# NVlabs/DREAM

Hardware: AMD Instinct MI355X
Metric: frames/s DREAM-vgg-q 400x400 b=128 inference (higher is better)
Workload: dtype f32

## Files before the change

dream_amd/csrc/conv_wino4.hip:

```cpp
#include <type_traits>
#include <stdlib.h>
#include <dream_cdna4.h>
#include "common.h"
#include "pack_device.h"
#include "../../include/dream_hip.h"

#ifndef DREAM_W4_DIAG
#define DREAM_W4_DIAG 0
#endif

namespace {

struct Wino4Params {
    const float *x;
    const float *u;
    const float *scale;
    const float *shift;
    const float *residual;
    float *y;
    float *y_full;
    int B, H, W, Cin, Cout, CoutPad;
    int TY, TX;
    int ntiles;
    int nblk, blk_per_xcd;
    unsigned long long magic_tpi, magic_tx;
    int flags;
    int out_scale, out_oy, out_ox;
    int in_scale, in_oy, in_ox;
    int stagger_n, stagger_unit;
    int ymap;
};

constexpr int W4T = 16;
constexpr int W4P = 36;
#ifndef DREAM_W4_RING
#define DREAM_W4_RING 8
#endif
#ifndef DREAM_W4_NARROW_RING
#define DREAM_W4_NARROW_RING 18
#endif
#ifndef DREAM_W4_PAT_RING
#define DREAM_W4_PAT_RING 10
#endif
#ifndef DREAM_W4_PAT_S1OFF
#define DREAM_W4_PAT_S1OFF 8
#endif
#ifndef DREAM_W4_S1
#define DREAM_W4_S1 10
#define DREAM_W4_S2 13
#define DREAM_W4_LX 3
#endif


template <bool NARROW>
struct W4Cfg {
    static constexpr int NW = NARROW ? 4 : 8;
    static constexpr int K = NARROW ? 8 : 16;
    static constexpr int Q = K / 4;
    static constexpr int KS = K / 4;
    static constexpr int PAD = 16 * NW;
    static constexpr int VPS = NARROW ? W4T * K : W4T * K + 16;
    static constexpr int VB = W4P * VPS;
    static constexpr int SROW = NARROW ? 14 : 25;
    static constexpr int QS = NARROW ? 7 : 6;
    static constexpr int SB = W4T * 6 * SROW * 4;
    static constexpr int RING = NARROW ? DREAM_W4_NARROW_RING : DREAM_W4_RING;
    static constexpr int AHEAD = RING - 2;
    static_assert(72 % RING == 0, "the weight ring must divide two chunks' positions");
    static constexpr bool PAIRS = NARROW && DREAM_W4_NARROW_PAIRS;
    static_assert(!PAIRS || RING % 2 == 0, "a ring of whole pairs");
    using vec = std::conditional_t<NARROW, f32x2, f32x4>;
};
template <bool NARROW>
DREAM_DEVICE int v4_slot(int q, int t) { return NARROW ? q ^ ((t >> 3) & 1) : q ^ ((t >> 2) & 2); }

DREAM_DEVICE f32x4 fma4(float c, f32x4 a, f32x4 b) {
    f32x4 r;
#pragma unroll
    for (int k = 0; k < 4; ++k) r[k] = __builtin_fmaf(c, a[k], b[k]);
    return r;
}

DREAM_DEVICE f32x4 sub4(f32x4 y, f32x4 x) { return pk_sub4(y, x); }
DREAM_DEVICE f32x4 bt_row(int j, const f32x4 *d) {
    switch (j) {
        case 0: return fma4(-2.0f, d[2], fma4(1.5f, sub4(d[3], d[1]), d[0] + d[4]));
        case 1: return fma4(2.5f, d[3], fma4(0.5f, d[2], sub4(d[4], d[1])));
        case 2: return fma4(0.5f, d[3], fma4(-2.5f, d[2], d[4] + d[1]));
        case 3: return fma4(2.0f, sub4(d[3], d[1]), sub4(d[4], d[2]));
        case 4: return fma4(-0.5f, sub4(d[3], d[1]), sub4(d[4], d[2]));
        default: return fma4(-2.0f, d[3], fma4(1.5f, sub4(d[4], d[2]), d[1] + d[5]));
    }
}

DREAM_DEVICE constexpr bool pat4_row_active(int pat, int i) { return pat == 0 || (((pat - 1) >> 1) == 0 ? i <= 4 : i >= 1); }
DREAM_DEVICE constexpr bool pat4_col_active(int pat, int j) { return pat == 0 || (((pat - 1) & 1) == 0 ? j <= 4 : j >= 1); }
DREAM_DEVICE constexpr bool pat4_active(int pat, int pp) { return pat4_row_active(pat, pp / 6) && pat4_col_active(pat, pp % 6); }
DREAM_DEVICE constexpr int pat4_count(int pat) { return pat == 0 ? 36 : 25; }
struct Pat4Table { int pos[36]; };
constexpr Pat4Table pat4_table(int pat) {
    Pat4Table t = {};
    int n = 0;
    for (int pp = 0; pp < 36; ++pp)
        if (pat4_active(pat, pp)) t.pos[n++] = pp;
    return t;
}
template <int PAT>
struct Pat4 { static constexpr Pat4Table table = pat4_table(PAT); };
#define pat4_pos(PAT, k) (Pat4<PAT>::table.pos[k])

template <int MODE, bool NARROW, int PAT = 0>
__global__ void __launch_bounds__(64 * W4Cfg<NARROW>::NW, 2) conv_wino4_kernel(const Wino4Params p) {
    using C = W4Cfg<NARROW>;
    using vec = typename C::vec;
    constexpr int W4K = C::K, W4NW = C::NW, V4PS = C::VPS, V4B = C::VB, S4ROW = C::SROW;
    constexpr int NPOS = pat4_count(PAT);
    constexpr int W4_RING = PAT ? DREAM_W4_PAT_RING : C::RING, W4_AHEAD = W4_RING - 2;
    static_assert((2 * NPOS) % W4_RING == 0, "the weight ring must divide two chunks' positions");
    DREAM_DYNAMIC_LDS(float, sV);
    const int tid = threadIdx.x;
    const int lane = tid & 63;
    const int wave = wave_index();
    const int item_id = wave * 48 + (lane < 48 ? lane : lane - 16);

    const int xcd = (int)(blockIdx.x & 7), J = (int)(gridDim.x >> 3);
    const int part = p.ymap ? xcd / p.ymap : xcd;
    const int blk_hi = (part + 1) * p.blk_per_xcd;
    const int blk_end = blk_hi < p.nblk ? blk_hi : p.nblk;
    int tb = part * p.blk_per_xcd + (int)(blockIdx.x >> 3);
    if (tb >= blk_end) return;
    const int n0 = (p.ymap ? xcd % p.ymap : (int)blockIdx.y) * (16 * W4NW);
    if (p.stagger_n > 1) {
        const unsigned w = blockIdx.x + blockIdx.y * gridDim.x;
        const int naps = (int)((w * 2654435761u >> 16) % (unsigned)p.stagger_n) * p.stagger_unit;
        for (int i = 0; i < naps; ++i) __builtin_amdgcn_s_sleep(127);
    }
    const int tiles_per_img = p.TY * p.TX;
    const int Si = PAT ? p.in_scale : 1;
    const size_t img_floats = (size_t)(Si * p.H) * (Si * p.W) * p.Cin;

    const int q1 = item_id % C::Q, r1 = (item_id / C::Q) % 6, t1 = (item_id / C::Q) / 6;
    const int s1_off = ((t1 * 6 + r1) * S4ROW + C::QS * q1) * 4;
    const int q2 = item_id % C::Q;
    const int j2 = NARROW ? (item_id >> 3) % 6 : (item_id >> 2) % 6;
    const int t2 = NARROW ? 4 * (item_id / 48) + ((item_id >> 1) & 3) : (item_id >> 2) / 6;
    const int s2_off = ((t2 * 6) * S4ROW + C::QS * q2 + j2) * 4;
    const int v2_off = j2 * V4PS + t2 * W4K + 4 * v4_slot<NARROW>(q2, t2);

    unsigned goff0;
    int item1 = t1 | (r1 << 8) | (q1 << 16);
    auto plan_item = [&](int tile0, int b0) {
        asm volatile("" : "+v"(item1));
        const int t = item1 & 255, r = (item1 >> 8) & 255, q = (item1 >> 16) & 255;
        const int tau = tile0 + t;
        const bool tv = tau < p.ntiles;
        const int b = div_magic40(tau, p.magic_tpi), rem = tau - b * tiles_per_img;
        const int ty = div_magic40(rem, p.magic_tx), tx = rem - ty * p.TX;
        const int gy = 4 * ty - 1 + r, x0 = 4 * tx - 1;
        const bool rok = tv & ((unsigned)gy < (unsigned)p.H);
        goff0 = PAT ? (unsigned)(((((b - b0) * Si * p.H + Si * gy + p.in_oy) * (Si * p.W) + Si * x0 + p.in_ox) * p.Cin + 4 * q) * 4)
                    : (unsigned)(((((b - b0) * p.H + gy) * p.W + x0) * p.Cin + 4 * q) * 4);
        item1 &= 0xffffff;
#pragma unroll
        for (int c = 0; c < 6; ++c) item1 |= (rok & ((unsigned)(x0 + c) < (unsigned)p.W)) ? (1 << (24 + c)) : 0;
    };
    const unsigned px_in = (unsigned)(Si * p.Cin * 4);
    auto item_offset = [&](int c) {
        if (DREAM_W4_DIAG & 16) {
            unsigned o = BUFFER_OOB;
            asm volatile("" : "+v"(o));
            return o;
        }
        return (item1 >> (24 + c)) & 1 ? goff0 + (unsigned)c * px_in : BUFFER_OOB;
    };
    auto block_tile0 = [&](int blk) { return blk < blk_end ? blk * W4T : p.ntiles; };
    auto block_xbuf = [&](int b0) {
        return make_buffer(p.x + (size_t)b0 * img_floats, ((size_t)(p.B - b0) * img_floats) * sizeof(float));
    };

    const int lt = lane & 15, lg = lane >> 4;
    const int a_off = NARROW ? lt * W4K + 4 * v4_slot<NARROW>(lg >> 1, lt) + 2 * (lg & 1) : lt * W4K + 4 * v4_slot<NARROW>(lg, lt);
    const unsigned b_lane = C::PAIRS ? (unsigned)(((wave * 16 + lt) * 16 + 4 * lg) * 4) : (unsigned)(((wave * 16 + lt) * W4K + C::KS * lg) * 4);
    const unsigned u_pos_stride = (unsigned)(p.CoutPad * W4K * 4);
    const BufferRsrc ubuf = make_buffer(p.u + (size_t)n0 * W4K, ((size_t)((p.Cin / W4K) * W4P + C::AHEAD) * p.CoutPad - (size_t)n0) * W4K * sizeof(float));

    f32x4 acc[W4P];
    const int nchunks = p.Cin / W4K;

    constexpr int BSTEP = C::PAIRS ? 2 : 1;
    std::conditional_t<C::PAIRS, f32x4, vec> bq[W4_RING / BSTEP];
    auto load_u = [&](unsigned soff) {
        if constexpr (C::PAIRS) return buffer_load_x4(ubuf, b_lane, soff);
        else if constexpr (NARROW) return buffer_load_x2(ubuf, b_lane, soff);
        else return buffer_load_x4(ubuf, b_lane, soff);
    };
#pragma unroll
    for (int k = 0; k < W4_AHEAD; k += BSTEP) bq[k / BSTEP] = load_u((unsigned)pat4_pos(PAT, k) * u_pos_stride);
    unsigned woff = (unsigned)W4_AHEAD * u_pos_stride;
    DREAM_OPAQUE_SGPR(woff);

    f32x4 *const sV4 = (f32x4 *)sV;
    vec *const sVa = (vec *)sV;
    int vrd[2], vwr[2], s1p = (2 * V4B + s1_off) / 4, s2p = (2 * V4B + s2_off) / 4;
#pragma unroll
    for (int h = 0; h < 2; ++h) {
        vrd[h] = (h * V4B + a_off) / C::KS;
        vwr[h] = (h * V4B + v2_off) / 4;
        asm volatile("" : "+v"(vrd[h]), "+v"(vwr[h]));
    }
    asm volatile("" : "+v"(s1p), "+v"(s2p));
    f32x4 d[6];
    auto pass1_piece = [&](int j) { sV4[s1p + j] = bt_row(j, d); };
    auto pass2_read = [&](int r) { d[r] = sV4[s2p + r * S4ROW]; };
    auto pass2_piece = [&](int i, int h) { if (pat4_row_active(PAT, i)) sV4[vwr[h] + i * (6 * V4PS / 4)] = bt_row(i, d); };

    vec a[2][2];
    auto read_a = [&](int set, int k, int h) {
        const int p0 = pat4_pos(PAT, k), p1 = pat4_pos(PAT, k + 1 < NPOS ? k + 1 : k);
        if constexpr (NARROW) {
            a[set][0] = lds_read_unmerged(sVa + vrd[h] + p0 * V4PS / C::KS);
            a[set][1] = lds_read_unmerged(sVa + vrd[h] + p1 * V4PS / C::KS);
        } else {
            a[set][0] = sVa[vrd[h] + p0 * V4PS / C::KS];
            if (k + 1 < NPOS) a[set][1] = sVa[vrd[h] + p1 * V4PS / C::KS];
        }
    };

    int tile0 = block_tile0(tb);
    int b0 = div_magic40(tile0, p.magic_tpi);
    BufferRsrc xbuf = block_xbuf(b0);
    plan_item(tile0, b0);
#pragma unroll
    for (int c = 0; c < 6; ++c) d[c] = buffer_load_x4(xbuf, item_offset(c), 0u);
#pragma unroll
    for (int j = 0; j < 6; ++j) pass1_piece(j);
    __syncthreads();
#pragma unroll
    for (int r = 0; r < 6; ++r) pass2_read(r);
#pragma unroll
    for (int i = 0; i < 6; ++i) pass2_piece(i, 0);
    __syncthreads();

    auto chunk = [&](auto ph_tag, bool last, int c, int tile0n, int b0n) __attribute__((always_inline)) {
        constexpr int PH = decltype(ph_tag)::value;
        constexpr int NSLOT = (NPOS + 1) / 2;
        constexpr int S1 = PAT ? NSLOT - DREAM_W4_PAT_S1OFF : DREAM_W4_S1, S2 = PAT ? S1 + 3 : DREAM_W4_S2;
        constexpr int LX = PAT ? 1 : DREAM_W4_LX;
        static_assert(LX <= S1, "the patch loads must be issued before pass 1");
        const unsigned coff = last ? 0u : (unsigned)((c + 1) * W4K * 4);
        const int cnext = last ? 0 : (c + 1) * W4P;
        if (PH == 1 && last) xbuf = block_xbuf(b0n);
        read_a(0, 0, PH);
        __builtin_amdgcn_sched_barrier(0);
#pragma unroll
        for (int s = 0; s < NSLOT; ++s) {
            const int k0 = 2 * s;
            const bool two = k0 + 1 < NPOS;
            const int pp = pat4_pos(PAT, k0), pp1 = pat4_pos(PAT, two ? k0 + 1 : k0);
            auto load_b = [&](int half) {
                if ((DREAM_W4_DIAG & 2) || (half && !two)) return;
                if (C::PAIRS && half) return;
                const int kn = k0 + half + W4_AHEAD;
                if constexpr (PAT == 0 && !(DREAM_W4_DIAG & 32)) {
                    if (kn == NPOS && last) woff = 0u;
                    bq[(PH * NPOS + kn) % W4_RING / BSTEP] = load_u(woff);
                    woff += BSTEP * u_pos_stride;
                    DREAM_OPAQUE_SGPR(woff);
                } else {
                    const int spos = kn >= NPOS ? cnext + pat4_pos(PAT, kn - NPOS) : c * W4P + pat4_pos(PAT, kn);
                    bq[(PH * NPOS + kn) % W4_RING / BSTEP] = load_u((DREAM_W4_DIAG & 32) ? 0u : (unsigned)spos * u_pos_stride);
                }
            };
            auto load_x = [&](int col) { if (!(DREAM_W4_DIAG & 1)) d[col] = buffer_load_x4(xbuf, item_offset(col), (DREAM_W4_DIAG & 64) ? 0u : coff); };
            auto pair = [&](int r) {
                const int i0 = (PH * NPOS + k0) % W4_RING, i1 = (PH * NPOS + k0 + 1) % W4_RING;
                if constexpr (C::PAIRS) {
                    acc[pp] = mfma_f32_16x16x4(a[s & 1][0][r], bq[i0 / 2][r], acc[pp]);
                    acc[pp1] = mfma_f32_16x16x4(a[s & 1][1][r], bq[i0 / 2][2 + r], acc[pp1]);
                } else {
                    acc[pp] = mfma_f32_16x16x4(a[s & 1][0][r], bq[i0][r], acc[pp]);
                    if (two) acc[pp1] = mfma_f32_16x16x4(a[s & 1][1][r], bq[i1][r], acc[pp1]);
                }
                __builtin_amdgcn_sched_barrier(0);
            };
            auto after = [&](int k) {
                if (k == 0) {
                    load_b(0);
                    if (s + 1 < NSLOT) read_a((s + 1) & 1, k0 + 2, PH);
                    if (PH == 1 && s == 0 && last) plan_item(tile0n, b0n);
                    if (s < LX) { for (int c2 = 0; c2 < 3 / LX; ++c2) load_x((6 / LX) * s + c2); }
                    if (!(DREAM_W4_DIAG & 8) && s >= S1 && s < S1 + 3) pass1_piece(2 * (s - S1));
                    if (!(DREAM_W4_DIAG & 8) && s == S2) { pass2_read(0); pass2_read(1); }
                    if (!(DREAM_W4_DIAG & 8) && s > S2 && s <= S2 + 3) pass2_piece(2 * (s - S2 - 1), 1 - PH);
                } else if (k == 1) {
                    load_b(1);
                    if (s < LX) { for (int c2 = 3 / LX; c2 < 6 / LX; ++c2) load_x((6 / LX) * s + c2); }
                    if (!(DREAM_W4_DIAG & 8) && s == S2) { pass2_read(2); pass2_read(3); }
                } else if (k == 2) {
                    if (!(DREAM_W4_DIAG & 8) && s >= S1 && s < S1 + 3) pass1_piece(2 * (s - S1) + 1);
                    if (!(DREAM_W4_DIAG & 8) && s == S2) { pass2_read(4); pass2_read(5); }
                    if (!(DREAM_W4_DIAG & 8) && s > S2 && s <= S2 + 3) pass2_piece(2 * (s - S2 - 1) + 1, 1 - PH);
                }
            };
            if constexpr (NARROW) {
                pair(0);
                after(0);
                after(1);
                pair(1);
                after(2);
            } else {
                pair(0);
                after(0);
                pair(1);
                after(1);
                pair(2);
                after(2);
                pair(3);
            }
            if (s == S1 + 2 && !(DREAM_W4_DIAG & 4)) {
                __builtin_amdgcn_sched_barrier(0);
            }
        }
        if (!(DREAM_W4_DIAG & 4)) __syncthreads();
    };
    const std::integral_constant<int, 0> ph0{};
    const std::integral_constant<int, 1> ph1{};

    constexpr bool pool = MODE == 1 || MODE == 4, both = MODE == 4, has_res = MODE == 2 || MODE == 3, mask = MODE == 3;
    auto epilogue = [&](auto site_tag, int tile0e, int b0e) {
        if (DREAM_W4_DIAG & 128) {
#pragma unroll
            for (int pp = 0; pp < W4P; ++pp)
                if (pat4_active(PAT, pp)) asm volatile("" :: "v"(acc[pp]));
            return;
        }
        const auto &e = *DREAM_KERNARG_SITE(p, decltype(site_tag)::value);
        const bool relu = (e.flags & DREAM_CONV_RELU) != 0;
        const bool late = MODE == 2 && (e.flags & DREAM_CONV_RES_AFTER_RELU) != 0;
        const int Ho = pool ? e.H / 2 : e.H, Wo = pool ? e.W / 2 : e.W, So = e.out_scale;
        const size_t out_img = (size_t)(So * Ho) * (So * Wo) * e.Cout;
        const unsigned px_b = (unsigned)(So * e.Cout * 4), row_b = (unsigned)(So * So * Wo * e.Cout * 4);
        const int ln = lane_id();
        const int lt = ln & 15, lg = ln >> 4;
        const int col = n0 + wave * 16 + lt;
        const bool cok = col < e.Cout;
        const float sc = (e.scale != nullptr && cok) ? e.scale[col] : 1.0f;
        const float sh = (e.shift != nullptr && cok) ? e.shift[col] : 0.0f;
        const BufferRsrc ybuf = make_buffer(e.y + (size_t)b0e * out_img, (DREAM_W4_DIAG & 256) ? 0 : (size_t)(e.B - b0e) * out_img * sizeof(float));
        const BufferRsrc rbuf = make_buffer(has_res ? e.residual + (size_t)b0e * out_img : e.y,
                                            has_res ? (size_t)(e.B - b0e) * out_img * sizeof(float) : 0);
        const size_t full_img = (size_t)e.H * e.W * e.Cout;
        const unsigned fpx_b = (unsigned)(e.Cout * 4), frow_b = (unsigned)(e.W * e.Cout * 4);
        const BufferRsrc fbuf = make_buffer(both ? e.y_full + (size_t)b0e * full_img : e.y, both ? (size_t)(e.B - b0e) * full_img * sizeof(float) : 0);
        const int tau0 = tile0e + lg * 4;
        int b = div_magic40(tau0, p.magic_tpi);
        const int rem = tau0 - b * tiles_per_img;
        int ty = div_magic40(rem, p.magic_tx), tx = rem - ty * p.TX;
        constexpr int NS = pool ? 2 : 4;
        unsigned basef[2][2];
        int limf[2][2];
        unsigned base4[2][2];
        int lim4[2][2];
        constexpr int FULL = pool ? 0x33 : 0xff;
#pragma unroll
        for (int rp = 0; rp < 2; ++rp)
#pragma unroll
            for (int h = 0; h < 2; ++h) {
                const bool tok = cok & ((tau0 + 2 * rp + h) < p.ntiles);
                const int oy = NS * ty, ox = NS * tx;
                base4[rp][h] = (unsigned)(((((b - b0e) * So * Ho + So * oy + e.out_oy) * (So * Wo) + So * ox + e.out_ox) * e.Cout + col) * 4);
                int m = 0;
#pragma unroll
                for (int i = 0; i < NS; ++i) m |= ((oy + i) < Ho ? 1 << i : 0) | ((ox + i) < Wo ? 16 << i : 0);
                lim4[rp][h] = tok ? m : 0;
                if (both) {
                    basef[rp][h] = (unsigned)(((((b - b0e) * e.H + 4 * ty) * e.W + 4 * tx) * e.Cout + col) * 4);
                    int mf = 0;
#pragma unroll
                    for (int i = 0; i < 4; ++i) mf |= ((4 * ty + i) < e.H ? 1 << i : 0) | ((4 * tx + i) < e.W ? 16 << i : 0);
                    limf[rp][h] = tok ? mf : 0;
                }
                const bool wrap_x = (tx + 1 == p.TX);
                const bool wrap_y = wrap_x & (ty + 1 == p.TY);
                tx = wrap_x ? 0 : tx + 1;
                ty = wrap_y ? 0 : (wrap_x ? ty + 1 : ty);
                b += wrap_y ? 1 : 0;
            }
        auto out_off4 = [&](int rp, int h, int i, int jj) {
            const bool inb = ((lim4[rp][h] >> i) & (lim4[rp][h] >> (4 + jj)) & 1) != 0;
            return inb ? base4[rp][h] + (unsigned)i * row_b + (unsigned)jj * px_b : BUFFER_OOB;
        };
        bool interior4[2];
#pragma unroll
        for (int rp = 0; rp < 2; ++rp) interior4[rp] = wave_all((lim4[rp][0] == FULL) & (lim4[rp][1] == FULL));
        auto load_col0 = [&](int rp, float (&r)[2][4]) {
            if (interior4[rp]) {
#pragma unroll
                for (int h = 0; h < 2; ++h)
#pragma unroll
                    for (int i = 0; i < 4; ++i) r[h][i] = buffer_load_f32(rbuf, base4[rp][h], (unsigned)i * row_b);
            } else {
#pragma unroll
                for (int h = 0; h < 2; ++h)
#pragma unroll
                    for (int i = 0; i < 4; ++i) r[h][i] = buffer_load_f32(rbuf, out_off4(rp, h, i, 0), 0u);
            }
        };
        float r0[2][4], r0n[2][4];
        if (has_res) load_col0(0, r0);
#pragma unroll
        for (int rp = 0; rp < 2; ++rp) {
            const unsigned (&base)[2] = base4[rp];
            auto out_off = [&](int h, int i, int jj) { return out_off4(rp, h, i, jj); };
            const bool all_interior = interior4[rp];
            auto fm = [](float c, f32x2 x, f32x2 y) { return __builtin_elementwise_fma(f32x2{c, c}, x, y); };
            f32x2 sA[6][4];
#pragma unroll
            for (int i = 0; i < 6; ++i) {
                f32x2 m[6];
#pragma unroll
                for (int j = 0; j < 6; ++j)
                    m[j] = pat4_active(PAT, 6 * i + j) ? f32x2{acc[6 * i + j][2 * rp], acc[6 * i + j][2 * rp + 1]} : f32x2{0.0f, 0.0f};
                const f32x2 t1 = pk_sub2(m[1], m[2]), t2 = m[1] + m[2];
                sA[i][0] = (m[0] + t2) + (m[3] + m[4]);
                sA[i][1] = fm(-2.0f, m[4], fm(0.5f, m[3], t1));
                sA[i][2] = fm(4.0f, m[4], fm(0.25f, m[3], t2));
                sA[i][3] = fm(-8.0f, m[4], fm(0.125f, m[3], t1)) + m[5];
            }
            auto finish = [&](float v, float rv) {
                if (has_res) v = mask ? (rv > 0.0f ? v : 0.0f) : (late ? v : v + rv);
                const float vr = fmaxf(v, 0.0f);
                v = relu ? vr : v;
                return (MODE == 2 && late) ? v + rv : v;
            };
            auto columns = [&](auto interior_tag, auto &rcur) {
                constexpr bool interior = decltype(interior_tag)::value;
                auto voff = [&](int h, int i, int j2) { return interior ? base[h] : out_off(h, i, j2); };
                auto soff = [&](int i, int j2) { return interior ? (unsigned)i * row_b + (unsigned)j2 * px_b : 0u; };
                float keep[2][2];
#pragma unroll
                for (int jj = 0; jj < 4; ++jj) {
                    float rnext[2][4];
                    if (has_res && jj == 3 && rp == 0) load_col0(1, r0n);
                    if (has_res && jj + 1 < 4) {
#pragma unroll
                        for (int h = 0; h < 2; ++h)
#pragma unroll
                            for (int i = 0; i < 4; ++i) rnext[h][i] = buffer_load_f32(rbuf, voff(h, i, jj + 1), soff(i, jj + 1));
                    }
                    const f32x2 t1 = pk_sub2(sA[1][jj], sA[2][jj]), t2 = sA[1][jj] + sA[2][jj];
                    f32x2 o4[4];
                    o4[0] = (sA[0][jj] + t2) + (sA[3][jj] + sA[4][jj]);
                    o4[1] = fm(-2.0f, sA[4][jj], fm(0.5f, sA[3][jj], t1));
                    o4[2] = fm(4.0f, sA[4][jj], fm(0.25f, sA[3][jj], t2));
                    o4[3] = fm(-8.0f, sA[4][jj], fm(0.125f, sA[3][jj], t1)) + sA[5][jj];
#pragma unroll
                    for (int i = 0; i < 4; ++i) o4[i] = o4[i] * f32x2{sc, sc} + f32x2{sh, sh};
#pragma unroll
                    for (int h = 0; h < 2; ++h) {
                        if (pool) {
                            float v[4];
#pragma unroll
                            for (int i = 0; i < 4; ++i) v[i] = finish(o4[i][h], 0.0f);
                            if (both) {
#pragma unroll
                                for (int i = 0; i < 4; ++i) {
                                    const bool inb = ((limf[rp][h] >> i) & (limf[rp][h] >> (4 + jj)) & 1) != 0;
                                    buffer_store_f32(fbuf, v[i], inb ? basef[rp][h] + (unsigned)i * frow_b + (unsigned)jj * fpx_b : BUFFER_OOB, 0u);
                                }
                            }
                            if ((jj & 1) == 0) {
                                keep[h][0] = fmaxf(v[0], v[1]);
                                keep[h][1] = fmaxf(v[2], v[3]);
                            } else {
                                buffer_store_f32(ybuf, fmaxf(keep[h][0], fmaxf(v[0], v[1])), voff(h, 0, jj >> 1), soff(0, jj >> 1));
                                buffer_store_f32(ybuf, fmaxf(keep[h][1], fmaxf(v[2], v[3])), voff(h, 1, jj >> 1), soff(1, jj >> 1));
                            }
                        } else {
#pragma unroll
                            for (int i = 0; i < 4; ++i)
                                buffer_store_f32(ybuf, finish(o4[i][h], has_res ? rcur[h][i] : 0.0f), voff(h, i, jj), soff(i, jj));
                        }
                    }
                    if (has_res && jj + 1 < 4) {
#pragma unroll
                        for (int h = 0; h < 2; ++h)
#pragma unroll
                            for (int i = 0; i < 4; ++i) rcur[h][i] = rnext[h][i];
                    }
                }
            };
            if (all_interior) columns(std::true_type{}, r0);
            else columns(std::false_type{}, r0);
            if (has_res && rp == 0) {
#pragma unroll
                for (int h = 0; h < 2; ++h)
#pragma unroll
                    for (int i = 0; i < 4; ++i) r0[h][i] = r0n[h][i];
            }
        }
    };

    auto run_blocks = [&]() __attribute__((always_inline)) {
        while (true) {
            const int tile0n = block_tile0(tb + J);
            const int b0n = div_magic40(tile0n, p.magic_tpi);
            const f32x4 zero = {0.0f, 0.0f, 0.0f, 0.0f};
#pragma unroll
            for (int pp = 0; pp < W4P; ++pp)
                if (pat4_active(PAT, pp)) acc[pp] = zero;
            for (int c = 0; c < nchunks; c += 2) {
                chunk(ph0, false, c, tile0n, b0n);
                chunk(ph1, c + 2 == nchunks, c + 1, tile0n, b0n);
            }
            epilogue(std::integral_constant<int, 0>{}, tile0, b0);
            tb += J;
            if (tb >= blk_end) break;
            tile0 = tile0n;
            b0 = b0n;
        }
    };
    run_blocks();
}

static_assert(W4Cfg<false>::K == 16 && W4Cfg<false>::PAD == 128 && W4Cfg<true>::K == 8 && W4Cfg<true>::PAD == 64 && W4P == 36,
              "pack_device.h assumes 16-channel chunks padded to 128 rows / 8-channel chunks padded to 64 rows, 36 positions");
__global__ void __launch_bounds__(256) wino4_pack_kernel(const float *w, float *u, int Cout, int Cin, int mode) {
    dream_pack::winograd4(w, u, Cout, Cin, mode, (int)blockIdx.x, (int)gridDim.x);
}

int g_max_workgroups4 = 0;
int g_stagger_n4 = -1, g_stagger_pct4 = 0;
int g_ymap4 = -1;

bool narrow_rows(int rows) { return rows <= W4Cfg<true>::PAD; }
struct PackShape { int k, rows_pad, ahead; };
PackShape pack_shape(int rows) {
    if (narrow_rows(rows)) return {W4Cfg<true>::K, W4Cfg<true>::PAD, W4Cfg<true>::AHEAD};
    return {W4Cfg<false>::K, (rows + W4Cfg<false>::PAD - 1) / W4Cfg<false>::PAD * W4Cfg<false>::PAD, W4Cfg<false>::AHEAD};
}

template <int MODE, bool NARROW, int PAT = 0>
int launch_wino4(const Wino4Params &p, void *stream) {
    using C = W4Cfg<NARROW>;
    void (*kernel)(const Wino4Params) = conv_wino4_kernel<MODE, NARROW, PAT>;
    const size_t lds = ((size_t)2 * C::VB + C::SB) * sizeof(float);
    if (dream_allow_full_lds((const void *)kernel)) return 2;
    const int ny = (p.Cout + 16 * C::NW - 1) / (16 * C::NW);
    const int resident = g_max_workgroups4 > 0 ? g_max_workgroups4 : (NARROW ? 512 : 256);
    Wino4Params q = p;
    dim3 grid;
    if (g_ymap4 && !NARROW && (ny == 2 || ny == 4) && resident >= 64 && p.nblk >= resident) {
        q.ymap = ny;
        q.blk_per_xcd = (p.nblk + 8 / ny - 1) / (8 / ny);
        grid = dim3((unsigned)(resident / 8 * 8), 1u);
    } else {
        int gx = resident / ny / 8 * 8;
        if (gx < 8) gx = 8;
        if (gx > (p.nblk + 7) / 8 * 8) gx = (p.nblk + 7) / 8 * 8;
        grid = dim3((unsigned)gx, (unsigned)ny);
    }
    hipLaunchKernelGGL(kernel, grid, dim3(64 * C::NW), lds, (hipStream_t)stream, q);
    DREAM_LAUNCH_OK();
    return 0;
}

template <bool NARROW>
int launch_wino4_mode(const Wino4Params &p, int mode, void *stream) {
    switch (mode) {
        case 0: return launch_wino4<0, NARROW>(p, stream);
        case 1: return launch_wino4<1, NARROW>(p, stream);
        case 2: return launch_wino4<2, NARROW>(p, stream);
        case 4: return launch_wino4<4, NARROW>(p, stream);
        default: return launch_wino4<3, NARROW>(p, stream);
    }
}

}

extern "C" size_t dream_conv3x3_winograd4_weight_floats(int rows, int cols) {
    const PackShape ps = pack_shape(rows);
    return ((size_t)(cols / ps.k) * W4P + ps.ahead) * ps.rows_pad * ps.k;
}

extern "C" int dream_conv3x3_winograd4_set_channel_block_pinning(int on) {
    DREAM_REQUIRE(on >= -1 && on <= 1, "winograd F(4x4): pinning %d", on);
    g_ymap4 = on;
    return 0;
}

extern "C" int dream_conv3x3_winograd4_set_stagger(int phases, int percent) {
    DREAM_REQUIRE(phases <= 1024 && percent >= 0 && percent <= 400, "winograd F(4x4): stagger %d phases over %d %%", phases, percent);
    g_stagger_n4 = phases < 0 ? -1 : (phases > 1 ? phases : 0);
    g_stagger_pct4 = percent;
    return 0;
}

extern "C" int dream_conv3x3_winograd4_set_max_workgroups(int n) {
    DREAM_REQUIRE(n >= 0, "winograd F(4x4): max workgroups %d", n);
    g_max_workgroups4 = n;
    return 0;
}

extern "C" int dream_pack_conv3x3_winograd4_weight(const float *w_oihw, float *u, int Cout, int Cin, int mode, void *stream) {
    DREAM_REQUIRE(w_oihw && u && Cout > 0 && Cin > 0 && (mode == 0 || mode == 1), "winograd F(4x4) pack: bad arguments");
    const int rows = mode == 0 ? Cout : Cin, cols = mode == 0 ? Cin : Cout;
    const PackShape ps = pack_shape(rows);
    DREAM_REQUIRE(cols % (2 * ps.k) == 0, "winograd F(4x4) pack: %d input channels, must be a multiple of %d", cols, 2 * ps.k);
    const size_t total = (size_t)(cols / ps.k) * ps.rows_pad * ps.k;
    size_t grid = (total + 255) / 256;
    if (grid > 4096) grid = 4096;
    hipLaunchKernelGGL(wino4_pack_kernel, dim3((unsigned)grid), dim3(256), 0, (hipStream_t)stream, w_oihw, u, Cout, Cin, mode);
    DREAM_LAUNCH_OK();
    if (dream_zero_words(u + (size_t)(cols / ps.k) * W4P * ps.rows_pad * ps.k, (size_t)ps.ahead * ps.rows_pad * ps.k * sizeof(float), (hipStream_t)stream))
        return 2;
    return 0;
}

namespace {

int wino4_setup(Wino4Params &p, const float *x, const float *u_packed, const float *scale, const float *shift, const float *residual,
                float *y, int B, int H, int W, int Cin, int Cout, int flags, int out_scale, int in_scale = 1) {
    DREAM_REQUIRE(x && u_packed && y, "winograd F(4x4) conv: null pointer");
    DREAM_REQUIRE(B > 0 && H > 0 && W > 0 && Cin > 0 && Cout > 0, "winograd F(4x4) conv: bad shape B=%d H=%d W=%d Cin=%d Cout=%d", B, H, W, Cin, Cout);
    const PackShape ps = pack_shape(Cout);
    DREAM_REQUIRE(Cin % (2 * ps.k) == 0, "winograd F(4x4) conv: Cin=%d must be a multiple of %d", Cin, 2 * ps.k);
    const size_t span_imgs = (size_t)W4T / ((size_t)((H + 3) / 4) * ((W + 3) / 4)) + 2;
    DREAM_REQUIRE(span_imgs * in_scale * in_scale * H * W * (size_t)Cin * sizeof(float) < ((size_t)1 << 31) &&
                  span_imgs * out_scale * out_scale * H * W * (size_t)Cout * sizeof(float) < ((size_t)1 << 31),
                  "winograd F(4x4) conv: image too large for 32-bit offsets");
    p.x = x; p.u = u_packed; p.scale = scale; p.shift = shift; p.residual = residual; p.y = y; p.y_full = nullptr;
    p.B = B; p.H = H; p.W = W; p.Cin = Cin; p.Cout = Cout;
    p.CoutPad = Cout <= ps.rows_pad ? ps.rows_pad : (Cout + ps.rows_pad - 1) / ps.rows_pad * ps.rows_pad;
    DREAM_REQUIRE(((size_t)(Cin / ps.k) * W4P + ps.ahead) * (size_t)p.CoutPad * ps.k * sizeof(float) < ((size_t)1 << 31), "winograd F(4x4) conv: weights too large");
    p.TY = (H + 3) / 4; p.TX = (W + 3) / 4;
    const long ntiles = (long)B * p.TY * p.TX;
    DREAM_REQUIRE(ntiles < ((long)1 << 24), "winograd F(4x4) conv: %ld tiles, the tile decomposition handles < 2^24", ntiles);
    p.ntiles = (int)ntiles;
    p.nblk = (p.ntiles + W4T - 1) / W4T;
    p.blk_per_xcd = (p.nblk + 7) / 8;
    p.magic_tpi = (((unsigned long long)1 << 40) + (unsigned long long)(p.TY * p.TX) - 1) / (unsigned long long)(p.TY * p.TX);
    p.magic_tx = (((unsigned long long)1 << 40) + (unsigned long long)p.TX - 1) / (unsigned long long)p.TX;
    p.flags = flags;
    p.out_scale = out_scale; p.out_oy = 0; p.out_ox = 0;
    p.in_scale = in_scale; p.in_oy = 0; p.in_ox = 0;
    p.ymap = 0;
    if (g_stagger_n4 < 0) {
        const char *e = getenv("DREAM_W4_STAGGER");
        int n = 0, pct = 0;
        if (e != nullptr && sscanf(e, "%d,%d", &n, &pct) != 2) { n = 0; pct = 0; }
        g_stagger_n4 = n > 1 ? n : 0;
        g_stagger_pct4 = pct;
    }
    {
        const double chunk_cycles = narrow_rows(Cout) ? 7000.0 : 13500.0;
        const double block_naps = (double)(Cin / ps.k) * chunk_cycles / 8128.0;
        p.stagger_n = g_stagger_n4;
        p.stagger_unit = g_stagger_n4 > 1 ? (int)(block_naps * g_stagger_pct4 / 100.0 / g_stagger_n4 + 0.5) : 0;
        if (p.stagger_n > 1 && p.stagger_unit < 1) p.stagger_unit = 1;
    }
    if (g_ymap4 < 0) {
        const char *e = getenv("DREAM_W4_YMAP");
        g_ymap4 = (e != nullptr && e[0] == '0') ? 0 : 1;
    }
    return 0;
}

}

extern "C" int dream_conv3x3_winograd4_nhwc_f32(const float *x, const float *u_packed, const float *scale, const float *shift,
                                                const float *residual, float *y, int B, int H, int W, int Cin, int Cout, int flags,
                                                void *stream) {
    DREAM_REQUIRE((flags & ~(DREAM_CONV_RELU | DREAM_CONV_POOL2 | DREAM_CONV_RELUMASK | DREAM_CONV_RES_AFTER_RELU)) == 0, "winograd F(4x4) conv: unsupported flags 0x%x", flags);
    DREAM_REQUIRE(!(flags & DREAM_CONV_RES_AFTER_RELU) || (residual != nullptr && !(flags & (DREAM_CONV_POOL2 | DREAM_CONV_RELUMASK))),
                  "winograd F(4x4) conv: residual-after-ReLU needs a residual and excludes the fused pool / the ReLU mask");
    DREAM_REQUIRE(!(flags & DREAM_CONV_POOL2) || (residual == nullptr && H >= 2 && W >= 2), "winograd F(4x4) conv: fused max-pool takes no residual");
    DREAM_REQUIRE(!(flags & DREAM_CONV_RELUMASK) || residual != nullptr, "winograd F(4x4) conv: ReLU mask without a mask tensor");
    Wino4Params p;
    if (int rc = wino4_setup(p, x, u_packed, scale, shift, residual, y, B, H, W, Cin, Cout, flags, 1)) return rc;
    const int mode = (flags & DREAM_CONV_POOL2) ? 1 : (flags & DREAM_CONV_RELUMASK) ? 3 : (residual != nullptr ? 2 : 0);
    return narrow_rows(Cout) ? launch_wino4_mode<true>(p, mode, stream) : launch_wino4_mode<false>(p, mode, stream);
}

extern "C" int dream_conv3x3_winograd4_pool_both_nhwc_f32(const float *x, const float *u_packed, const float *scale, const float *shift,
                                                          float *y_full, float *y_pool, int B, int H, int W, int Cin, int Cout, int flags,
                                                          void *stream) {
    DREAM_REQUIRE((flags & ~DREAM_CONV_RELU) == 0, "winograd F(4x4) conv + pool: unsupported flags 0x%x", flags);
    DREAM_REQUIRE(y_full != nullptr && y_pool != nullptr && H >= 2 && W >= 2, "winograd F(4x4) conv + pool: null output or map too small");
    Wino4Params p;
    if (int rc = wino4_setup(p, x, u_packed, scale, shift, nullptr, y_pool, B, H, W, Cin, Cout, flags, 1)) return rc;
    p.y_full = y_full;
    return narrow_rows(Cout) ? launch_wino4_mode<true>(p, 4, stream) : launch_wino4_mode<false>(p, 4, stream);
}

extern "C" size_t dream_convT4x4_winograd4_weight_floats(int Cout, int Cin) { return 4 * dream_conv3x3_winograd4_weight_floats(Cout, Cin); }

extern "C" int dream_pack_convT4x4_winograd4_weight(const float *wT, float *u4, float *scratch, int Cin, int Cout, int mode, void *stream) {
    DREAM_REQUIRE(wT && u4 && scratch && Cin > 0 && Cout > 0 && (mode == 0 || mode == 1), "winograd F(4x4) convT pack: bad arguments");
    if (int rc = dream_convT4x4_phase_weights(wT, scratch, Cin, Cout, mode, stream)) return rc;
    const int rows = mode == 0 ? Cout : Cin, cols = mode == 0 ? Cin : Cout;
    const size_t per_u = dream_conv3x3_winograd4_weight_floats(rows, cols);
    for (int ph = 0; ph < 4; ++ph)
        if (int rc = dream_pack_conv3x3_winograd4_weight(scratch + (size_t)ph * Cout * Cin * 9, u4 + ph * per_u, rows, cols, 0, stream)) return rc;
    return 0;
}

extern "C" int dream_conv4x4s2_winograd4_nhwc_f32(const float *dy, const float *u4, float *dx, int B, int H, int W, int Cout, int Cin,
                                                  void *stream) {
    DREAM_REQUIRE(Cin > 64, "winograd F(4x4) conv4x4s2: needs more than 64 output channels (the wide workgroup shape), got %d", Cin);
    Wino4Params p;
    if (int rc = wino4_setup(p, dy, u4, nullptr, nullptr, nullptr, dx, B, H, W, Cout, Cin, 0, 1, 2)) return rc;
    const size_t per_u = dream_conv3x3_winograd4_weight_floats(Cin, Cout);
    for (int ph = 0; ph < 4; ++ph) {
        p.u = u4 + ph * per_u;
        p.in_oy = ph >> 1; p.in_ox = ph & 1;
        p.residual = ph == 0 ? nullptr : dx;
        int rc;
        switch (ph) {
            case 0: rc = launch_wino4<0, false, 4>(p, stream); break;
            case 1: rc = launch_wino4<2, false, 3>(p, stream); break;
            case 2: rc = launch_wino4<2, false, 2>(p, stream); break;
            default: rc = launch_wino4<2, false, 1>(p, stream); break;
        }
        if (rc) return rc;
    }
    return 0;
}

extern "C" int dream_conv_transpose4x4s2_winograd4_nhwc_f32(const float *x, const float *u4, const float *scale, const float *shift,
                                                            float *y, int B, int H, int W, int Cin, int Cout, int flags, void *stream) {
    DREAM_REQUIRE((flags & ~DREAM_CONV_RELU) == 0, "winograd F(4x4) convT: unsupported flags 0x%x", flags);
    DREAM_REQUIRE(Cout > 64, "winograd F(4x4) convT: needs more than 64 output channels (the wide workgroup shape), got %d", Cout);
    Wino4Params p;
    if (int rc = wino4_setup(p, x, u4, scale, shift, nullptr, y, B, H, W, Cin, Cout, flags, 2)) return rc;
    const size_t per_u = dream_conv3x3_winograd4_weight_floats(Cout, Cin);
    for (int ph = 0; ph < 4; ++ph) {
        p.u = u4 + ph * per_u;
        p.out_oy = ph >> 1; p.out_ox = ph & 1;
        int rc;
        switch (ph) {
            case 0: rc = launch_wino4<0, false, 1>(p, stream); break;
            case 1: rc = launch_wino4<0, false, 2>(p, stream); break;
            case 2: rc = launch_wino4<0, false, 3>(p, stream); break;
            default: rc = launch_wino4<0, false, 4>(p, stream); break;
        }
        if (rc) return rc;
    }
    return 0;
}
```

Before: 2658.

## Transpose MFMA operands so each lane holds four channels and store 16-byte vectors

The MFMA operands are swapped so the accumulator comes out transposed. Each lane now holds four consecutive output channels of one tile, instead of four tiles of one channel. The epilogue is rewritten around this layout: one tile-index decode per lane, per-lane scale/shift vectors, and dwordx4 buffer loads and stores of residuals and outputs whenever Cout and the pointers are 16-byte aligned, with a scalar fallback otherwise. This is meant to cut the number of memory instructions and the address arithmetic in the epilogue, at the cost of more live registers (sA for both channel pairs) and reliance on b_lane for the lane mapping.

```diff
diff --git a/dream_amd/csrc/conv_wino4.hip b/dream_amd/csrc/conv_wino4.hip
--- a/dream_amd/csrc/conv_wino4.hip
+++ b/dream_amd/csrc/conv_wino4.hip
@@ -275,11 +275,11 @@
             auto pair = [&](int r) {
                 const int i0 = (PH * NPOS + k0) % W4_RING, i1 = (PH * NPOS + k0 + 1) % W4_RING;
                 if constexpr (C::PAIRS) {
-                    acc[pp] = mfma_f32_16x16x4(a[s & 1][0][r], bq[i0 / 2][r], acc[pp]);
-                    acc[pp1] = mfma_f32_16x16x4(a[s & 1][1][r], bq[i0 / 2][2 + r], acc[pp1]);
+                    acc[pp] = mfma_f32_16x16x4(bq[i0 / 2][r], a[s & 1][0][r], acc[pp]);
+                    acc[pp1] = mfma_f32_16x16x4(bq[i0 / 2][2 + r], a[s & 1][1][r], acc[pp1]);
                 } else {
-                    acc[pp] = mfma_f32_16x16x4(a[s & 1][0][r], bq[i0][r], acc[pp]);
-                    if (two) acc[pp1] = mfma_f32_16x16x4(a[s & 1][1][r], bq[i1][r], acc[pp1]);
+                    acc[pp] = mfma_f32_16x16x4(bq[i0][r], a[s & 1][0][r], acc[pp]);
+                    if (two) acc[pp1] = mfma_f32_16x16x4(bq[i1][r], a[s & 1][1][r], acc[pp1]);
                 }
                 __builtin_amdgcn_sched_barrier(0);
             };
@@ -340,165 +340,184 @@
         const int Ho = pool ? e.H / 2 : e.H, Wo = pool ? e.W / 2 : e.W, So = e.out_scale;
         const size_t out_img = (size_t)(So * Ho) * (So * Wo) * e.Cout;
         const unsigned px_b = (unsigned)(So * e.Cout * 4), row_b = (unsigned)(So * So * Wo * e.Cout * 4);
-        const int ln = lane_id();
-        const int lt = ln & 15, lg = ln >> 4;
-        const int col = n0 + wave * 16 + lt;
-        const bool cok = col < e.Cout;
-        const float sc = (e.scale != nullptr && cok) ? e.scale[col] : 1.0f;
-        const float sh = (e.shift != nullptr && cok) ? e.shift[col] : 0.0f;
+        unsigned bl = b_lane;
+        asm volatile("" : "+v"(bl));
+        const int lrow = (int)(bl >> 2) / (C::PAIRS ? 4 : C::KS);
+        const int lt = (lrow >> 2) & 15, lg = lrow & 3;
+        const int c0 = n0 + wave * 16 + 4 * lg;
+        const bool vec16 = ((e.Cout & 3) == 0) & ((((size_t)e.y | (has_res ? (size_t)e.residual : (size_t)0) | (both ? (size_t)e.y_full : (size_t)0)) & 15) == 0);
+        int cmask = 0;
+        f32x4 sc, sh;
+#pragma unroll
+        for (int k = 0; k < 4; ++k) {
+            const bool ck = c0 + k < e.Cout;
+            cmask |= ck ? 1 << k : 0;
+            sc[k] = (e.scale != nullptr && ck) ? e.scale[c0 + k] : 1.0f;
+            sh[k] = (e.shift != nullptr && ck) ? e.shift[c0 + k] : 0.0f;
+        }
         const BufferRsrc ybuf = make_buffer(e.y + (size_t)b0e * out_img, (DREAM_W4_DIAG & 256) ? 0 : (size_t)(e.B - b0e) * out_img * sizeof(float));
         const BufferRsrc rbuf = make_buffer(has_res ? e.residual + (size_t)b0e * out_img : e.y,
                                             has_res ? (size_t)(e.B - b0e) * out_img * sizeof(float) : 0);
         const size_t full_img = (size_t)e.H * e.W * e.Cout;
         const unsigned fpx_b = (unsigned)(e.Cout * 4), frow_b = (unsigned)(e.W * e.Cout * 4);
         const BufferRsrc fbuf = make_buffer(both ? e.y_full + (size_t)b0e * full_img : e.y, both ? (size_t)(e.B - b0e) * full_img * sizeof(float) : 0);
-        const int tau0 = tile0e + lg * 4;
-        int b = div_magic40(tau0, p.magic_tpi);
-        const int rem = tau0 - b * tiles_per_img;
-        int ty = div_magic40(rem, p.magic_tx), tx = rem - ty * p.TX;
+        const int tau = tile0e + lt;
+        const int b = div_magic40(tau, p.magic_tpi);
+        const int rem = tau - b * tiles_per_img;
+        const int ty = div_magic40(rem, p.magic_tx), tx = rem - ty * p.TX;
         constexpr int NS = pool ? 2 : 4;
-        unsigned basef[2][2];
-        int limf[2][2];
-        unsigned base4[2][2];
-        int lim4[2][2];
         constexpr int FULL = pool ? 0x33 : 0xff;
-#pragma unroll
-        for (int rp = 0; rp < 2; ++rp)
-#pragma unroll
-            for (int h = 0; h < 2; ++h) {
-                const bool tok = cok & ((tau0 + 2 * rp + h) < p.ntiles);
-                const int oy = NS * ty, ox = NS * tx;
-                base4[rp][h] = (unsigned)(((((b - b0e) * So * Ho + So * oy + e.out_oy) * (So * Wo) + So * ox + e.out_ox) * e.Cout + col) * 4);
-                int m = 0;
-#pragma unroll
-                for (int i = 0; i < NS; ++i) m |= ((oy + i) < Ho ? 1 << i : 0) | ((ox + i) < Wo ? 16 << i : 0);
-                lim4[rp][h] = tok ? m : 0;
-                if (both) {
-                    basef[rp][h] = (unsigned)(((((b - b0e) * e.H + 4 * ty) * e.W + 4 * tx) * e.Cout + col) * 4);
-                    int mf = 0;
-#pragma unroll
-                    for (int i = 0; i < 4; ++i) mf |= ((4 * ty + i) < e.H ? 1 << i : 0) | ((4 * tx + i) < e.W ? 16 << i : 0);
-                    limf[rp][h] = tok ? mf : 0;
-                }
-                const bool wrap_x = (tx + 1 == p.TX);
-                const bool wrap_y = wrap_x & (ty + 1 == p.TY);
-                tx = wrap_x ? 0 : tx + 1;
-                ty = wrap_y ? 0 : (wrap_x ? ty + 1 : ty);
-                b += wrap_y ? 1 : 0;
-            }
-        auto out_off4 = [&](int rp, int h, int i, int jj) {
-            const bool inb = ((lim4[rp][h] >> i) & (lim4[rp][h] >> (4 + jj)) & 1) != 0;
-            return inb ? base4[rp][h] + (unsigned)i * row_b + (unsigned)jj * px_b : BUFFER_OOB;
+        const bool tok = (c0 < e.Cout) & (tau < p.ntiles);
+        const int oy = NS * ty, ox = NS * tx;
+        const unsigned base = (unsigned)(((((b - b0e) * So * Ho + So * oy + e.out_oy) * (So * Wo) + So * ox + e.out_ox) * e.Cout + c0) * 4);
+        int lim = 0;
+#pragma unroll
+        for (int i = 0; i < NS; ++i) lim |= ((oy + i) < Ho ? 1 << i : 0) | ((ox + i) < Wo ? 16 << i : 0);
+        lim = tok ? lim : 0;
+        unsigned basef = 0;
+        int limf = 0;
+        if (both) {
+            basef = (unsigned)(((((b - b0e) * e.H + 4 * ty) * e.W + 4 * tx) * e.Cout + c0) * 4);
+#pragma unroll
+            for (int i = 0; i < 4; ++i) limf |= ((4 * ty + i) < e.H ? 1 << i : 0) | ((4 * tx + i) < e.W ? 16 << i : 0);
+            limf = tok ? limf : 0;
+        }
+        auto out_off = [&](int i, int jj) {
+            const bool inb = ((lim >> i) & (lim >> (4 + jj)) & 1) != 0;
+            return inb ? base + (unsigned)i * row_b + (unsigned)jj * px_b : BUFFER_OOB;
         };
-        bool interior4[2];
-#pragma unroll
-        for (int rp = 0; rp < 2; ++rp) interior4[rp] = wave_all((lim4[rp][0] == FULL) & (lim4[rp][1] == FULL));
-        auto load_col0 = [&](int rp, float (&r)[2][4]) {
-            if (interior4[rp]) {
-#pragma unroll
-                for (int h = 0; h < 2; ++h)
-#pragma unroll
-                    for (int i = 0; i < 4; ++i) r[h][i] = buffer_load_f32(rbuf, base4[rp][h], (unsigned)i * row_b);
-            } else {
-#pragma unroll
-                for (int h = 0; h < 2; ++h)
-#pragma unroll
-                    for (int i = 0; i < 4; ++i) r[h][i] = buffer_load_f32(rbuf, out_off4(rp, h, i, 0), 0u);
+        const bool all_interior = wave_all(lim == FULL);
+        auto load4 = [&](auto vec_tag, unsigned vo, unsigned so) {
+            if constexpr (decltype(vec_tag)::value) return buffer_load_x4(rbuf, vo, so);
+            else {
+                f32x4 r;
+#pragma unroll
+                for (int k = 0; k < 4; ++k) r[k] = buffer_load_f32(rbuf, vo, so + 4u * (unsigned)k);
+                return r;
             }
         };
-        float r0[2][4], r0n[2][4];
-        if (has_res) load_col0(0, r0);
-#pragma unroll
-        for (int rp = 0; rp < 2; ++rp) {
-            const unsigned (&base)[2] = base4[rp];
-            auto out_off = [&](int h, int i, int jj) { return out_off4(rp, h, i, jj); };
-            const bool all_interior = interior4[rp];
-            auto fm = [](float c, f32x2 x, f32x2 y) { return __builtin_elementwise_fma(f32x2{c, c}, x, y); };
-            f32x2 sA[6][4];
-#pragma unroll
-            for (int i = 0; i < 6; ++i) {
+        auto store4 = [&](auto vec_tag, const BufferRsrc &buf, f32x4 v, unsigned vo, unsigned so) {
+            if constexpr (decltype(vec_tag)::value) buffer_store_x4(buf, v, vo, so);
+            else {
+#pragma unroll
+                for (int k = 0; k < 4; ++k) buffer_store_f32(buf, v[k], (cmask >> k) & 1 ? vo + 4u * (unsigned)k : BUFFER_OOB, so);
+            }
+        };
+        f32x4 rcur[4];
+        auto load_col0 = [&]() {
+            if (vec16 && all_interior) {
+#pragma unroll
+                for (int i = 0; i < 4; ++i) rcur[i] = load4(std::true_type{}, base, (unsigned)i * row_b);
+            } else if (vec16) {
+#pragma unroll
+                for (int i = 0; i < 4; ++i) rcur[i] = load4(std::true_type{}, out_off(i, 0), 0u);
+            } else {
+#pragma unroll
+                for (int i = 0; i < 4; ++i) rcur[i] = load4(std::false_type{}, out_off(i, 0), 0u);
+            }
+        };
+        auto fm = [](float c, f32x2 x, f32x2 y) { return __builtin_elementwise_fma(f32x2{c, c}, x, y); };
+        f32x2 sA[2][6][4];
+#pragma unroll
+        for (int i = 0; i < 6; ++i)
+#pragma unroll
+            for (int cp = 0; cp < 2; ++cp) {
                 f32x2 m[6];
 #pragma unroll
                 for (int j = 0; j < 6; ++j)
-                    m[j] = pat4_active(PAT, 6 * i + j) ? f32x2{acc[6 * i + j][2 * rp], acc[6 * i + j][2 * rp + 1]} : f32x2{0.0f, 0.0f};
+                    m[j] = pat4_active(PAT, 6 * i + j) ? f32x2{acc[6 * i + j][2 * cp], acc[6 * i + j][2 * cp + 1]} : f32x2{0.0f, 0.0f};
                 const f32x2 t1 = pk_sub2(m[1], m[2]), t2 = m[1] + m[2];
-                sA[i][0] = (m[0] + t2) + (m[3] + m[4]);
-                sA[i][1] = fm(-2.0f, m[4], fm(0.5f, m[3], t1));
-                sA[i][2] = fm(4.0f, m[4], fm(0.25f, m[3], t2));
-                sA[i][3] = fm(-8.0f, m[4], fm(0.125f, m[3], t1)) + m[5];
+                sA[cp][i][0] = (m[0] + t2) + (m[3] + m[4]);
+                sA[cp][i][1] = fm(-2.0f, m[4], fm(0.5f, m[3], t1));
+                sA[cp][i][2] = fm(4.0f, m[4], fm(0.25f, m[3], t2));
+                sA[cp][i][3] = fm(-8.0f, m[4], fm(0.125f, m[3], t1)) + m[5];
+                if (has_res && i == 1 && cp == 1) load_col0();
             }
-            auto finish = [&](float v, float rv) {
-                if (has_res) v = mask ? (rv > 0.0f ? v : 0.0f) : (late ? v : v + rv);
-                const float vr = fmaxf(v, 0.0f);
-                v = relu ? vr : v;
-                return (MODE == 2 && late) ? v + rv : v;
-            };
-            auto columns = [&](auto interior_tag, auto &rcur) {
-                constexpr bool interior = decltype(interior_tag)::value;
-                auto voff = [&](int h, int i, int j2) { return interior ? base[h] : out_off(h, i, j2); };
-                auto soff = [&](int i, int j2) { return interior ? (unsigned)i * row_b + (unsigned)j2 * px_b : 0u; };
-                float keep[2][2];
-#pragma unroll
-                for (int jj = 0; jj < 4; ++jj) {
-                    float rnext[2][4];
-                    if (has_res && jj == 3 && rp == 0) load_col0(1, r0n);
-                    if (has_res && jj + 1 < 4) {
-#pragma unroll
-                        for (int h = 0; h < 2; ++h)
-#pragma unroll
-                            for (int i = 0; i < 4; ++i) rnext[h][i] = buffer_load_f32(rbuf, voff(h, i, jj + 1), soff(i, jj + 1));
+        auto finish = [&](float v, float rv) {
+            if (has_res) v = mask ? (rv > 0.0f ? v : 0.0f) : (late ? v : v + rv);
+            const float vr = fmaxf(v, 0.0f);
+            v = relu ? vr : v;
+            return (MODE == 2 && late) ? v + rv : v;
+        };
+        auto finish4 = [&](f32x4 v, f32x4 rv) {
+            f32x4 r;
+#pragma unroll
+            for (int k = 0; k < 4; ++k) r[k] = finish(v[k], rv[k]);
+            return r;
+        };
+        auto max4 = [](f32x4 x, f32x4 y) {
+            f32x4 r;
+#pragma unroll
+            for (int k = 0; k < 4; ++k) r[k] = fmaxf(x[k], y[k]);
+            return r;
+        };
+        auto columns = [&](auto interior_tag, auto vec_tag) {
+            constexpr bool interior = decltype(interior_tag)::value;
+            auto voff = [&](int i, int j2) { return interior ? base : out_off(i, j2); };
+            auto soff = [&](int i, int j2) { return interior ? (unsigned)i * row_b + (unsigned)j2 * px_b : 0u; };
+            auto st_voff = [&](int i, int j2) { return interior ? base + ((unsigned)i * row_b + (unsigned)j2 * px_b) : out_off(i, j2); };
+            const f32x4 zero4 = {0.0f, 0.0f, 0.0f, 0.0f};
+            f32x4 keep[2];
+#pragma unroll
+            for (int jj = 0; jj < 4; ++jj) {
+                constexpr bool ahead = decltype(vec_tag)::value;
+                f32x4 rnext[4];
+                if (has_res && ahead && jj + 1 < 4) {
+#pragma unroll
+                    for (int i = 0; i < 4; ++i) rnext[i] = load4(vec_tag, voff(i, jj + 1), soff(i, jj + 1));
+                }
+                if (has_res && !ahead && jj > 0) {
+#pragma unroll
+                    for (int i = 0; i < 4; ++i) rcur[i] = load4(vec_tag, voff(i, jj), soff(i, jj));
+                }
+                f32x4 o[4];
+#pragma unroll
+                for (int cp = 0; cp < 2; ++cp) {
+                    const f32x2 (&s)[6][4] = sA[cp];
+                    const f32x2 t1 = pk_sub2(s[1][jj], s[2][jj]), t2 = s[1][jj] + s[2][jj];
+                    f32x2 o4[4];
+                    o4[0] = (s[0][jj] + t2) + (s[3][jj] + s[4][jj]);
+                    o4[1] = fm(-2.0f, s[4][jj], fm(0.5f, s[3][jj], t1));
+                    o4[2] = fm(4.0f, s[4][jj], fm(0.25f, s[3][jj], t2));
+                    o4[3] = fm(-8.0f, s[4][jj], fm(0.125f, s[3][jj], t1)) + s[5][jj];
+#pragma unroll
+                    for (int i = 0; i < 4; ++i) {
+                        o4[i] = o4[i] * f32x2{sc[2 * cp], sc[2 * cp + 1]} + f32x2{sh[2 * cp], sh[2 * cp + 1]};
+                        o[i][2 * cp] = o4[i][0];
+                        o[i][2 * cp + 1] = o4[i][1];
                     }
-                    const f32x2 t1 = pk_sub2(sA[1][jj], sA[2][jj]), t2 = sA[1][jj] + sA[2][jj];
-                    f32x2 o4[4];
-                    o4[0] = (sA[0][jj] + t2) + (sA[3][jj] + sA[4][jj]);
-                    o4[1] = fm(-2.0f, sA[4][jj], fm(0.5f, sA[3][jj], t1));
-                    o4[2] = fm(4.0f, sA[4][jj], fm(0.25f, sA[3][jj], t2));
-                    o4[3] = fm(-8.0f, sA[4][jj], fm(0.125f, sA[3][jj], t1)) + sA[5][jj];
-#pragma unroll
-                    for (int i = 0; i < 4; ++i) o4[i] = o4[i] * f32x2{sc, sc} + f32x2{sh, sh};
-#pragma unroll
-                    for (int h = 0; h < 2; ++h) {
-                        if (pool) {
-                            float v[4];
-#pragma unroll
-                            for (int i = 0; i < 4; ++i) v[i] = finish(o4[i][h], 0.0f);
-                            if (both) {
-#pragma unroll
-                                for (int i = 0; i < 4; ++i) {
-                                    const bool inb = ((limf[rp][h] >> i) & (limf[rp][h] >> (4 + jj)) & 1) != 0;
-                                    buffer_store_f32(fbuf, v[i], inb ? basef[rp][h] + (unsigned)i * frow_b + (unsigned)jj * fpx_b : BUFFER_OOB, 0u);
-                                }
-                            }
-                            if ((jj & 1) == 0) {
-                                keep[h][0] = fmaxf(v[0], v[1]);
-                                keep[h][1] = fmaxf(v[2], v[3]);
-                            } else {
-                                buffer_store_f32(ybuf, fmaxf(keep[h][0], fmaxf(v[0], v[1])), voff(h, 0, jj >> 1), soff(0, jj >> 1));
-                                buffer_store_f32(ybuf, fmaxf(keep[h][1], fmaxf(v[2], v[3])), voff(h, 1, jj >> 1), soff(1, jj >> 1));
-                            }
-                        } else {
-#pragma unroll
-                            for (int i = 0; i < 4; ++i)
-                                buffer_store_f32(ybuf, finish(o4[i][h], has_res ? rcur[h][i] : 0.0f), voff(h, i, jj), soff(i, jj));
+                }
+                if (pool) {
+                    f32x4 v[4];
+#pragma unroll
+                    for (int i = 0; i < 4; ++i) v[i] = finish4(o[i], zero4);
+                    if (both) {
+#pragma unroll
+                        for (int i = 0; i < 4; ++i) {
+                            const bool inb = ((limf >> i) & (limf >> (4 + jj)) & 1) != 0;
+                            store4(vec_tag, fbuf, v[i], inb ? basef + (unsigned)i * frow_b + (unsigned)jj * fpx_b : BUFFER_OOB, 0u);
                         }
                     }
-                    if (has_res && jj + 1 < 4) {
-#pragma unroll
-                        for (int h = 0; h < 2; ++h)
-#pragma unroll
-                            for (int i = 0; i < 4; ++i) rcur[h][i] = rnext[h][i];
+                    if ((jj & 1) == 0) {
+                        keep[0] = max4(v[0], v[1]);
+                        keep[1] = max4(v[2], v[3]);
+                    } else {
+                        store4(vec_tag, ybuf, max4(keep[0], max4(v[0], v[1])), st_voff(0, jj >> 1), 0u);
+                        store4(vec_tag, ybuf, max4(keep[1], max4(v[2], v[3])), st_voff(1, jj >> 1), 0u);
                     }
+                } else {
+#pragma unroll
+                    for (int i = 0; i < 4; ++i) store4(vec_tag, ybuf, finish4(o[i], has_res ? rcur[i] : zero4), st_voff(i, jj), 0u);
                 }
-            };
-            if (all_interior) columns(std::true_type{}, r0);
-            else columns(std::false_type{}, r0);
-            if (has_res && rp == 0) {
-#pragma unroll
-                for (int h = 0; h < 2; ++h)
-#pragma unroll
-                    for (int i = 0; i < 4; ++i) r0[h][i] = r0n[h][i];
+                if (has_res && ahead && jj + 1 < 4) {
+#pragma unroll
+                    for (int i = 0; i < 4; ++i) rcur[i] = rnext[i];
+                }
             }
-        }
+        };
+        if (vec16 && all_interior) columns(std::true_type{}, std::true_type{});
+        else if (vec16) columns(std::false_type{}, std::true_type{});
+        else columns(std::false_type{}, std::false_type{});
     };
 
     auto run_blocks = [&]() __attribute__((always_inline)) {
```

After: 2642. Within noise of the previous version (-0.6%).
